# OpenDriveLab/OccNet

Hardware: AMD Instinct MI355X
Metric: nuScenes samples/sec (6-cam 900x1600 -> 200x200x16 voxels) (higher is better)
Workload: dtype f32 hot path (GEMM operands bf16x3-split, SCA value rows q16 block floating point) + bf16 backbone; 1 GPU; bevformer_base_occ forward: 6x(3x928x1600) images -> ResNet-50+FPN -> 4 BEVFormer layers (TSA+SCA+FFN) -> lifter + 2xConv3d decoder -> 200x200x16 voxels x (17 logits + 2 flow); history_frames=0, mode=infer, scope=e2e, input=resident-f32, samples_per_gpu=1, global_batch=1, parallelism=dp1, step_graph=False, linear_precision=bf16x3, backbone_dtype=bf16

## Files before the change

### occnet_amd/csrc/bottleneck64_nhwc_bf16.hip

```cpp
#include "common.h"

namespace occ {

constexpr int kBnTH = 8, kBnTW = 16, kBnHH = 10, kBnHW = 18, kBnNP = kBnHH * kBnHW;
constexpr int kBnXS = 80;
constexpr int kBnXA = 192 * kBnXS;
constexpr int kBnMS = 144;
constexpr int kBnH1ROW = kBnHW * kBnMS;
constexpr int kBnH1 = kBnHH * kBnH1ROW;
constexpr int kBnC2 = 128 * kBnMS;
constexpr int kBnOLD = 256 + 4;

__global__ void mfma_pack_b_frag_kernel(const float* __restrict__ w, unsigned short* __restrict__ packed,
                                        int N, int K) {
  const long n_el = (long)N * K;
  const long idx = (long)blockIdx.x * blockDim.x + threadIdx.x;
  if (idx >= n_el) return;
  const int j = (int)(idx & 7), lane = (int)((idx >> 3) & 63);
  const long rest = idx >> 9;
  const int nts = N / 32;
  const int nt = (int)(rest % nts), ks = (int)(rest / nts);
  const int n = nt * 32 + (lane & 31), k = ks * 16 + (lane >> 5) * 8 + j;
  packed[idx] = bf16_rne(w[(long)n * K + k]);
}

template <int CIN, bool DS>
__global__ __launch_bounds__(256, 2) void bottleneck64_nhwc_bf16_kernel(
    const uint4* __restrict__ x, const uint4* __restrict__ w1p, const float* __restrict__ b1,
    const uint4* __restrict__ w2p, const float* __restrict__ b2, const uint4* __restrict__ w3p,
    const float* __restrict__ b3, unsigned short* __restrict__ out, int H, int W, int tiles_x, int tiles_y) {
  static_assert(CIN % 32 == 0 && (!DS || CIN == 64), "downsample variant keeps both x chunks in LDS");
  constexpr int NCH = CIN / 32, CQ = CIN / 8;
  constexpr int STAGE_BYTES = 2 * kBnXA + kBnH1 + kBnC2;
  __shared__ __attribute__((aligned(16))) char lds[STAGE_BYTES];
  static_assert(32 * kBnOLD * 4 <= 2 * kBnXA + kBnH1, "epilogue transpose aliases the x chunks + c1 halo");
  char* const sH1 = lds + 2 * kBnXA;
  char* const sC2 = sH1 + kBnH1;
  const int tid = threadIdx.x, lane = tid & 63, wave = tid >> 6;
  const int vi = lane & 31, kb = lane >> 5;
  int bid = blockIdx.x;
  const int tx_i = bid % tiles_x; bid /= tiles_x;
  const int ty_i = bid % tiles_y;
  const int img = bid / tiles_y;
  const int y0 = ty_i * kBnTH, x0 = tx_i * kBnTW;

  long hofs0, hofs1, hofs2;
  int hdst0, hdst1, hdst2;
  bool hin0, hin1, hin2, hlive0, hlive1, hlive2;
#define OCC_BN_ROLE(K, OFS, DST, IN, LIVE)                                                        \
  {                                                                                               \
    const int idx = tid + 256 * (K);                                                              \
    LIVE = idx < kBnNP * 4;                                                                       \
    const int p = LIVE ? idx >> 2 : 0, piece = idx & 3;                                           \
    const int hy = p / kBnHW, hx = p % kBnHW;                                                     \
    const int iy = y0 - 1 + hy, ix = x0 - 1 + hx;                                                 \
    IN = LIVE && iy >= 0 && iy < H && ix >= 0 && ix < W;                                          \
    const int cy = min(max(iy, 0), H - 1), cx = min(max(ix, 0), W - 1);                           \
    OFS = (((long)img * H + cy) * W + cx) * CQ + piece;                                           \
    DST = p * kBnXS + piece * 16;                                                                 \
  }
  OCC_BN_ROLE(0, hofs0, hdst0, hin0, hlive0)
  OCC_BN_ROLE(1, hofs1, hdst1, hin1, hlive1)
  OCC_BN_ROLE(2, hofs2, hdst2, hin2, hlive2)
#undef OCC_BN_ROLE
  const unsigned hm0 = hin0 ? 0xffffffffu : 0u, hm1 = hin1 ? 0xffffffffu : 0u, hm2 = hin2 ? 0xffffffffu : 0u;
  uint4 vh0_0, vh1_0, vh2_0, vh0_1, vh1_1, vh2_1, vh0_2, vh1_2, vh2_2, vh0_3, vh1_3, vh2_3;
#define OCC_BN_ISSUE_X(S, CH)                                                                     \
  {                                                                                               \
    const long cq = (long)(CH) * 4;                                                               \
    vh0_##S = x[hofs0 + cq]; vh1_##S = x[hofs1 + cq]; vh2_##S = x[hofs2 + cq];                    \
  }
  const int rot = DS ? 0 : (int)((blockIdx.x * 5u) % (unsigned)NCH);
#define OCC_BN_CH(CI) (((CI) + rot) % NCH)

  const int ntA = wave & 1, mtA0 = 3 * (wave >> 1);
  const int ntB = wave & 1, mtB0 = 2 * (wave >> 1);
  float4 bA[4], bB[4];
#pragma unroll
  for (int g = 0; g < 4; ++g) {
    bA[g] = *reinterpret_cast<const float4*>(b1 + ntA * 32 + 8 * g + 4 * kb);
    bB[g] = *reinterpret_cast<const float4*>(b2 + ntB * 32 + 8 * g + 4 * kb);
  }
  f32x16 acc1[3];
#pragma unroll
  for (int j = 0; j < 3; ++j)
#pragma unroll
    for (int r = 0; r < 16; ++r) acc1[j][r] = 0.f;
  uint4 wa[4][2];
#define OCC_BN_ISSUE_W1(SLOT, CH)                                                                 \
  {                                                                                               \
    wa[SLOT][0] = w1p[(((long)(CH) * 2 + 0) * 2 + ntA) * 64 + lane];                              \
    wa[SLOT][1] = w1p[(((long)(CH) * 2 + 1) * 2 + ntA) * 64 + lane];                              \
  }
#define OCC_BN_ISSUE_XW(S, CH) { OCC_BN_ISSUE_W1(S, CH) OCC_BN_ISSUE_X(S, CH) }
  OCC_BN_ISSUE_XW(0, OCC_BN_CH(0))
  OCC_BN_ISSUE_XW(1, OCC_BN_CH(NCH > 1 ? 1 : 0))
  if (NCH > 2) {
    OCC_BN_ISSUE_XW(2, OCC_BN_CH(NCH > 2 ? 2 : 0))
    OCC_BN_ISSUE_XW(3, OCC_BN_CH(NCH > 3 ? 3 : 0))
  }
#define OCC_BN_STEP_A(S, CI)                                                                      \
  {                                                                                               \
    char* sX = lds + ((CI) & 1) * kBnXA;                                                          \
    if (hlive0) *reinterpret_cast<uint4*>(sX + hdst0) = make_uint4(vh0_##S.x & hm0, vh0_##S.y & hm0, vh0_##S.z & hm0, vh0_##S.w & hm0); \
    if (hlive1) *reinterpret_cast<uint4*>(sX + hdst1) = make_uint4(vh1_##S.x & hm1, vh1_##S.y & hm1, vh1_##S.z & hm1, vh1_##S.w & hm1); \
    if (hlive2) *reinterpret_cast<uint4*>(sX + hdst2) = make_uint4(vh2_##S.x & hm2, vh2_##S.y & hm2, vh2_##S.z & hm2, vh2_##S.w & hm2); \
    const bf16x8 wf0 = __builtin_bit_cast(bf16x8, wa[S][0]), wf1 = __builtin_bit_cast(bf16x8, wa[S][1]); \
    __syncthreads();                                                                              \
    if ((CI) + 4 < NCH) OCC_BN_ISSUE_XW(S, OCC_BN_CH((CI) + 4 < NCH ? (CI) + 4 : NCH - 1))        \
    _Pragma("unroll") for (int j = 0; j < 3; ++j) {                                               \
      const bf16x8 af0 = *reinterpret_cast<const bf16x8*>(sX + ((mtA0 + j) * 32 + vi) * kBnXS + kb * 16);      \
      const bf16x8 af1 = *reinterpret_cast<const bf16x8*>(sX + ((mtA0 + j) * 32 + vi) * kBnXS + 32 + kb * 16); \
      acc1[j] = __builtin_amdgcn_mfma_f32_32x32x16_bf16(wf0, af0, acc1[j], 0, 0, 0);              \
      acc1[j] = __builtin_amdgcn_mfma_f32_32x32x16_bf16(wf1, af1, acc1[j], 0, 0, 0);              \
    }                                                                                             \
  }
#pragma unroll
  for (int ci = 0; ci < NCH; ci += 4) {
    OCC_BN_STEP_A(0, ci)
    if (ci + 1 < NCH) OCC_BN_STEP_A(1, ci + 1)
    if (ci + 2 < NCH) OCC_BN_STEP_A(2, ci + 2)
    if (ci + 3 < NCH) OCC_BN_STEP_A(3, ci + 3)
  }
#undef OCC_BN_STEP_A
#undef OCC_BN_ISSUE_XW
#undef OCC_BN_ISSUE_W1
#undef OCC_BN_ISSUE_X
#undef OCC_BN_CH

  constexpr int PFB = 12;
  uint4 wr[PFB];
#pragma unroll
  for (int s = 0; s < PFB; ++s) wr[s] = w2p[((long)s * 2 + ntB) * 64 + lane];

#pragma unroll
  for (int j = 0; j < 3; ++j) {
    const int p = (mtA0 + j) * 32 + vi;
    const int hy = p / kBnHW, hx = p - hy * kBnHW;
    const int iy = y0 - 1 + hy, ix = x0 - 1 + hx;
    const float m = (iy >= 0 && iy < H && ix >= 0 && ix < W) ? 1.f : 0.f;
    if (p < kBnNP) {
      char* dst = sH1 + p * kBnMS + (ntA * 32 + 4 * kb) * 2;
#pragma unroll
      for (int g = 0; g < 4; ++g) {
        const float v0 = fmaxf(acc1[j][4 * g + 0] + bA[g].x, 0.f) * m, v1 = fmaxf(acc1[j][4 * g + 1] + bA[g].y, 0.f) * m;
        const float v2 = fmaxf(acc1[j][4 * g + 2] + bA[g].z, 0.f) * m, v3 = fmaxf(acc1[j][4 * g + 3] + bA[g].w, 0.f) * m;
        *reinterpret_cast<uint2*>(dst + 16 * g) = make_uint2(pack_bf16x2_rne(v0, v1), pack_bf16x2_rne(v2, v3));
      }
    }
  }
  __syncthreads();

  f32x16 acc2[2];
#pragma unroll
  for (int j = 0; j < 2; ++j)
#pragma unroll
    for (int r = 0; r < 16; ++r) acc2[j][r] = 0.f;
  const int ab0 = (2 * mtB0 + (vi >> 4)) * kBnH1ROW + (vi & 15) * kBnMS + kb * 16;
  const int ab1 = ab0 + 2 * kBnH1ROW;
  {
    bf16x8 a0 = *reinterpret_cast<const bf16x8*>(sH1 + ab0), a1 = *reinterpret_cast<const bf16x8*>(sH1 + ab1);
#pragma unroll
    for (int s = 0; s < 36; ++s) {
      const bf16x8 wf = __builtin_bit_cast(bf16x8, wr[s % PFB]);
      if (s + PFB < 36) wr[s % PFB] = w2p[((long)(s + PFB) * 2 + ntB) * 64 + lane];
      bf16x8 a0n = a0, a1n = a1;
      if (s + 1 < 36) {
        const int tap = (s + 1) >> 2, ks = (s + 1) & 3;
        const int toff = (tap / 3) * kBnH1ROW + (tap % 3) * kBnMS + ks * 32;
        a0n = *reinterpret_cast<const bf16x8*>(sH1 + ab0 + toff);
        a1n = *reinterpret_cast<const bf16x8*>(sH1 + ab1 + toff);
      }
      acc2[0] = __builtin_amdgcn_mfma_f32_32x32x16_bf16(wf, a0, acc2[0], 0, 0, 0);
      acc2[1] = __builtin_amdgcn_mfma_f32_32x32x16_bf16(wf, a1, acc2[1], 0, 0, 0);
      __builtin_amdgcn_sched_barrier(0);
      a0 = a0n; a1 = a1n;
    }
  }
  constexpr int KS3 = DS ? 8 : 4;
  uint4 w3r[4][2];
#define OCC_BN_ISSUE_W3(SLOT, KS)                                                                 \
  {                                                                                               \
    w3r[SLOT][0] = w3p[((long)(KS) * 8 + 2 * wave + 0) * 64 + lane];                              \
    w3r[SLOT][1] = w3p[((long)(KS) * 8 + 2 * wave + 1) * 64 + lane];                              \
  }
  OCC_BN_ISSUE_W3(0, 0)
  OCC_BN_ISSUE_W3(1, 1)
  OCC_BN_ISSUE_W3(2, 2)
  OCC_BN_ISSUE_W3(3, 3)
#pragma unroll
  for (int j = 0; j < 2; ++j) {
    char* dst = sC2 + ((mtB0 + j) * 32 + vi) * kBnMS + (ntB * 32 + 4 * kb) * 2;
#pragma unroll
    for (int g = 0; g < 4; ++g) {
      const float v0 = fmaxf(acc2[j][4 * g + 0] + bB[g].x, 0.f), v1 = fmaxf(acc2[j][4 * g + 1] + bB[g].y, 0.f);
      const float v2 = fmaxf(acc2[j][4 * g + 2] + bB[g].z, 0.f), v3 = fmaxf(acc2[j][4 * g + 3] + bB[g].w, 0.f);
      *reinterpret_cast<uint2*>(dst + 16 * g) = make_uint2(pack_bf16x2_rne(v0, v1), pack_bf16x2_rne(v2, v3));
    }
  }
  __syncthreads();

  f32x16 acc3[4][2];
#pragma unroll
  for (int rt = 0; rt < 4; ++rt)
#pragma unroll
    for (int t = 0; t < 2; ++t)
#pragma unroll
      for (int r = 0; r < 16; ++r) acc3[rt][t][r] = 0.f;
#pragma unroll
  for (int ks = 0; ks < KS3; ++ks) {
    const bf16x8 wf0 = __builtin_bit_cast(bf16x8, w3r[ks & 3][0]);
    const bf16x8 wf1 = __builtin_bit_cast(bf16x8, w3r[ks & 3][1]);
    if (ks + 4 < KS3) OCC_BN_ISSUE_W3(ks & 3, ks + 4)
#pragma unroll
    for (int rt = 0; rt < 4; ++rt) {
      bf16x8 af;
      if (ks < 4) {
        af = *reinterpret_cast<const bf16x8*>(sC2 + (rt * 32 + vi) * kBnMS + ks * 32 + kb * 16);
      } else {
        const int p = (2 * rt + (vi >> 4) + 1) * kBnHW + (vi & 15) + 1;
        af = *reinterpret_cast<const bf16x8*>(lds + ((ks - 4) >> 1) * kBnXA + p * kBnXS + ((ks - 4) & 1) * 32 + kb * 16);
      }
      acc3[rt][0] = __builtin_amdgcn_mfma_f32_32x32x16_bf16(af, wf0, acc3[rt][0], 0, 0, 0);
      acc3[rt][1] = __builtin_amdgcn_mfma_f32_32x32x16_bf16(af, wf1, acc3[rt][1], 0, 0, 0);
    }
  }
#undef OCC_BN_ISSUE_W3

  const int c = lane * 4;
  const float4 bv = *reinterpret_cast<const float4*>(b3 + c);
  float* sO = reinterpret_cast<float*>(lds);
  const unsigned short* xs = reinterpret_cast<const unsigned short*>(x);
  uint2 rv[8], rn[8];
#define OCC_BN_ISSUE_RES(DST, RT)                                                                 \
  _Pragma("unroll") for (int rr = 0; rr < 8; ++rr) {                                              \
    DST[rr] = make_uint2(0u, 0u);                                                                 \
    if (!DS) {                                                                                    \
      const int row = wave * 8 + rr;                                                              \
      const int cy = min(y0 + 2 * (RT) + (row >> 4), H - 1), cx = min(x0 + (row & 15), W - 1);    \
      DST[rr] = *reinterpret_cast<const uint2*>(xs + (((long)img * H + cy) * W + cx) * CIN + c);  \
    }                                                                                             \
  }
  OCC_BN_ISSUE_RES(rn, 0)
#pragma unroll
  for (int rt = 0; rt < 4; ++rt) {
    __syncthreads();
#pragma unroll
    for (int t = 0; t < 2; ++t)
#pragma unroll
      for (int r = 0; r < 16; ++r)
        sO[((r & 3) + 8 * (r >> 2) + 4 * kb) * kBnOLD + (wave * 2 + t) * 32 + vi] = acc3[rt][t][r];
#pragma unroll
    for (int rr = 0; rr < 8; ++rr) rv[rr] = rn[rr];
    if (rt + 1 < 4) OCC_BN_ISSUE_RES(rn, rt + 1)
    __syncthreads();
#pragma unroll
    for (int rr = 0; rr < 8; ++rr) {
      const int row = wave * 8 + rr;
      const int oy = y0 + 2 * rt + (row >> 4), ox = x0 + (row & 15);
      if (oy < H && ox < W) {
        float4 v = *reinterpret_cast<const float4*>(sO + row * kBnOLD + c);
        v.x += bv.x + bf16_to_f32((unsigned short)(rv[rr].x & 0xffffu));
        v.y += bv.y + bf16_to_f32((unsigned short)(rv[rr].x >> 16));
        v.z += bv.z + bf16_to_f32((unsigned short)(rv[rr].y & 0xffffu));
        v.w += bv.w + bf16_to_f32((unsigned short)(rv[rr].y >> 16));
        v.x = fmaxf(v.x, 0.f); v.y = fmaxf(v.y, 0.f); v.z = fmaxf(v.z, 0.f); v.w = fmaxf(v.w, 0.f);
        const uint2 o = make_uint2(pack_bf16x2_rne(v.x, v.y), pack_bf16x2_rne(v.z, v.w));
        *reinterpret_cast<uint2*>(out + (((long)img * H + oy) * W + ox) * 256 + c) = o;
      }
    }
  }
#undef OCC_BN_ISSUE_RES
}

}

extern "C" int occ_mfma_pack_b_frag_bf16(const float* weight, void* packed, int N, int K, void* stream) {
  using namespace occ;
  OCC_CHECK_ARG(weight && packed, "mfma_pack_b_frag_bf16: null pointer argument");
  OCC_CHECK_ARG(N > 0 && K > 0, "mfma_pack_b_frag_bf16: bad dimension");
  if (N % 32 || K % 16) {
    set_error("mfma_pack_b_frag_bf16: N=%d K=%d (need N %% 32 == 0, K %% 16 == 0)", N, K);
    return OCC_E_UNSUPPORTED;
  }
  const long n = (long)N * K;
  hipLaunchKernelGGL(mfma_pack_b_frag_kernel, dim3((unsigned)((n + 255) / 256)), dim3(256), 0,
                     reinterpret_cast<hipStream_t>(stream), weight, reinterpret_cast<unsigned short*>(packed),
                     N, K);
  OCC_CHECK_LAUNCH("mfma_pack_b_frag_bf16");
  return OCC_OK;
}

extern "C" int occ_bottleneck64_nhwc_bf16(const void* x, const void* w1_frag, const float* b1,
                                          const void* w2_frag, const float* b2, const void* w3_frag,
                                          const float* b3, void* out, int batch, int H, int W, int Cin,
                                          int downsample, void* stream) {
  using namespace occ;
  OCC_CHECK_ARG(x && w1_frag && b1 && w2_frag && b2 && w3_frag && b3 && out,
                "bottleneck64_nhwc_bf16: null pointer argument");
  OCC_CHECK_ARG(batch > 0 && H > 0 && W > 0, "bottleneck64_nhwc_bf16: bad dimension");
  if (!((Cin == 256 && !downsample) || (Cin == 64 && downsample))) {
    set_error("bottleneck64_nhwc_bf16: no kernel for Cin=%d downsample=%d (256/identity or 64/projection)", Cin,
              downsample);
    return OCC_E_UNSUPPORTED;
  }
  const int tiles_x = (W + kBnTW - 1) / kBnTW, tiles_y = (H + kBnTH - 1) / kBnTH;
  hipStream_t st = reinterpret_cast<hipStream_t>(stream);
  const unsigned gx = (unsigned)((long)batch * tiles_x * tiles_y);
#define OCC_BN_LAUNCH(CINN, DSS)                                                                     \
  hipLaunchKernelGGL((bottleneck64_nhwc_bf16_kernel<CINN, DSS>), dim3(gx), dim3(256), 0, st,            \
                     reinterpret_cast<const uint4*>(x), reinterpret_cast<const uint4*>(w1_frag), b1,    \
                     reinterpret_cast<const uint4*>(w2_frag), b2, reinterpret_cast<const uint4*>(w3_frag), \
                     b3, reinterpret_cast<unsigned short*>(out), H, W, tiles_x, tiles_y)
  if (downsample) OCC_BN_LAUNCH(64, true); else OCC_BN_LAUNCH(256, false);
#undef OCC_BN_LAUNCH
  OCC_CHECK_LAUNCH("bottleneck64_nhwc_bf16");
  return OCC_OK;
}
```

### occnet_amd/csrc/common.h

```cpp
#pragma once
#include <hip/hip_runtime.h>
#include <stdint.h>
#include <stdio.h>
#include <stdlib.h>
#include "../../include/occnet_amd.h"

namespace occ {

void set_error(const char* fmt, ...);
#define OCC_CHECK_ARG(cond, ...)              \
  do {                                        \
    if (!(cond)) {                            \
      ::occ::set_error(__VA_ARGS__);          \
      return OCC_E_INVALID;                   \
    }                                         \
  } while (0)
#define OCC_CHECK_LAUNCH(what)                                                  \
  do {                                                                          \
    hipError_t e__ = hipGetLastError();                                         \
    if (e__ != hipSuccess) {                                                    \
      ::occ::set_error("%s: launch failed: %s", what, hipGetErrorString(e__));  \
      return OCC_E_LAUNCH;                                                      \
    }                                                                           \
  } while (0)
// ... 107 lines not shown
  __builtin_amdgcn_wave_barrier();
  __builtin_amdgcn_fence(__ATOMIC_ACQUIRE, "wavefront");
}

template <int UNROLL>
__device__ __forceinline__ float4 gather_samples(const float* __restrict__ vb,
                                                 const SampleParam* sp, int ns, float4 acc) {
  int s = 0;
  for (; s + UNROLL <= ns; s += UNROLL) {
    float4 w[UNROLL];
    int4 o[UNROLL];
#pragma unroll
    for (int u = 0; u < UNROLL; ++u) {
      w[u] = *reinterpret_cast<const float4*>(sp[s + u].w);
      o[u] = *reinterpret_cast<const int4*>(sp[s + u].o);
    }
    float4 v[UNROLL][4];
#pragma unroll
    for (int u = 0; u < UNROLL; ++u) {
      v[u][0] = *reinterpret_cast<const float4*>(vb + o[u].x);
      v[u][1] = *reinterpret_cast<const float4*>(vb + o[u].y);
      v[u][2] = *reinterpret_cast<const float4*>(vb + o[u].z);
      v[u][3] = *reinterpret_cast<const float4*>(vb + o[u].w);
    }
#pragma unroll
    for (int u = 0; u < UNROLL; ++u) {
      const float ww[4] = {w[u].x, w[u].y, w[u].z, w[u].w};
#pragma unroll
      for (int k = 0; k < 4; ++k) {
        acc.x = fmaf(ww[k], v[u][k].x, acc.x);
        acc.y = fmaf(ww[k], v[u][k].y, acc.y);
        acc.z = fmaf(ww[k], v[u][k].z, acc.z);
        acc.w = fmaf(ww[k], v[u][k].w, acc.w);
      }
    }
  }
  for (; s < ns; ++s) {
    const float4 w = *reinterpret_cast<const float4*>(sp[s].w);
    const int4 o = *reinterpret_cast<const int4*>(sp[s].o);
    const float4 v0 = *reinterpret_cast<const float4*>(vb + o.x);
    const float4 v1 = *reinterpret_cast<const float4*>(vb + o.y);
    const float4 v2 = *reinterpret_cast<const float4*>(vb + o.z);
    const float4 v3 = *reinterpret_cast<const float4*>(vb + o.w);
    acc.x = fmaf(w.x, v0.x, acc.x); acc.y = fmaf(w.x, v0.y, acc.y);
    acc.z = fmaf(w.x, v0.z, acc.z); acc.w = fmaf(w.x, v0.w, acc.w);
    acc.x = fmaf(w.y, v1.x, acc.x); acc.y = fmaf(w.y, v1.y, acc.y);
    acc.z = fmaf(w.y, v1.z, acc.z); acc.w = fmaf(w.y, v1.w, acc.w);
    acc.x = fmaf(w.z, v2.x, acc.x); acc.y = fmaf(w.z, v2.y, acc.y);
    acc.z = fmaf(w.z, v2.z, acc.z); acc.w = fmaf(w.z, v2.w, acc.w);
    acc.x = fmaf(w.w, v3.x, acc.x); acc.y = fmaf(w.w, v3.y, acc.y);
    acc.z = fmaf(w.w, v3.z, acc.z); acc.w = fmaf(w.w, v3.w, acc.w);
  }
  return acc;
}

constexpr unsigned kOobOffset = 0x7fffff00u;

struct __attribute__((aligned(16))) SampleParamB {
  float w[4];
  unsigned o[4];
};

__device__ __forceinline__ int bilinear_setup_b(float loc_x, float loc_y, float attn, int H, int W, int lvl_pix0,
                                                unsigned pix_bytes, unsigned dead, int live, SampleParamB& sp) {
  const BilinearTerms t = bilinear_terms(loc_x, loc_y, H, W, live);
  const int base = lvl_pix0 + t.h_low * W + t.w_low;
  sp.w[0] = t.c[0] ? t.hh * t.hw * attn : 0.f; sp.o[0] = t.c[0] ? (unsigned)base * pix_bytes : dead;
  sp.w[1] = t.c[1] ? t.hh * t.lw * attn : 0.f; sp.o[1] = t.c[1] ? (unsigned)(base + 1) * pix_bytes : dead;
  sp.w[2] = t.c[2] ? t.lh * t.hw * attn : 0.f; sp.o[2] = t.c[2] ? (unsigned)(base + W) * pix_bytes : dead;
  sp.w[3] = t.c[3] ? t.lh * t.lw * attn : 0.f; sp.o[3] = t.c[3] ? (unsigned)(base + W + 1) * pix_bytes : dead;
  return t.c[0] + t.c[1] + t.c[2] + t.c[3];
}

__device__ __forceinline__ __amdgpu_buffer_rsrc_t uniform_rsrc(const void* base, unsigned bytes) {
  const unsigned long long a = reinterpret_cast<unsigned long long>(base);
  const unsigned lo = __builtin_amdgcn_readfirstlane((unsigned)a);
  const unsigned hi = __builtin_amdgcn_readfirstlane((unsigned)(a >> 32));
  void* p = reinterpret_cast<void*>(((unsigned long long)hi << 32) | lo);
  return __builtin_amdgcn_make_buffer_rsrc(p, 0, (int)__builtin_amdgcn_readfirstlane(bytes), 0x00020000);
}

__device__ __forceinline__ void block_lds_sync() { asm volatile("s_waitcnt lgkmcnt(0)\n\ts_barrier" ::: "memory"); }

__device__ __forceinline__ float4 buf_load16(__amdgpu_buffer_rsrc_t rsrc, unsigned byte_off) {
  return __builtin_bit_cast(float4, __builtin_amdgcn_raw_buffer_load_b128(rsrc, (int)byte_off, 0, 0));
}

__device__ __forceinline__ void fma4(float4& acc, float w, const float4& v) {
  acc.x = fmaf(w, v.x, acc.x); acc.y = fmaf(w, v.y, acc.y);
  acc.z = fmaf(w, v.z, acc.z); acc.w = fmaf(w, v.w, acc.w);
}

template <int UNROLL>
__device__ __forceinline__ float4 gather_samples_buf(__amdgpu_buffer_rsrc_t rsrc, unsigned lane_off,
                                                     const SampleParamB* sp, int ns, float4 acc) {
  int s = 0;
  for (; s + UNROLL <= ns; s += UNROLL) {
    float4 v[UNROLL][4];
#pragma unroll
    for (int u = 0; u < UNROLL; ++u) {
      const occ_u32x4 o = *reinterpret_cast<const occ_u32x4*>(sp[s + u].o);
#pragma unroll
      for (int k = 0; k < 4; ++k) v[u][k] = buf_load16(rsrc, o[k] + lane_off);
    }
#pragma unroll
    for (int u = 0; u < UNROLL; ++u) {
      const float4 w = *reinterpret_cast<const float4*>(sp[s + u].w);
      fma4(acc, w.x, v[u][0]); fma4(acc, w.y, v[u][1]); fma4(acc, w.z, v[u][2]); fma4(acc, w.w, v[u][3]);
    }
  }
  for (; s < ns; ++s) {
    const occ_u32x4 o = *reinterpret_cast<const occ_u32x4*>(sp[s].o);
    const float4 w = *reinterpret_cast<const float4*>(sp[s].w);
    float4 v[4];
#pragma unroll
    for (int k = 0; k < 4; ++k) v[k] = buf_load16(rsrc, o[k] + lane_off);
    fma4(acc, w.x, v[0]); fma4(acc, w.y, v[1]); fma4(acc, w.z, v[2]); fma4(acc, w.w, v[3]);
  }
  return acc;
}

__device__ __forceinline__ void fma_mix_lo(float& acc, float w, unsigned packed) {
  asm("v_fma_mix_f32 %0, %1, %2, %0 op_sel_hi:[0,1,0]" : "+v"(acc) : "v"(w), "v"(packed));
}
__device__ __forceinline__ void fma_mix_hi(float& acc, float w, unsigned packed) {
  asm("v_fma_mix_f32 %0, %1, %2, %0 op_sel:[0,1,0] op_sel_hi:[0,1,0]" : "+v"(acc) : "v"(w), "v"(packed));
}

__device__ __forceinline__ void fma8h(float4& acc, float4& acc2, float w, const float4& raw) {
  const occ_u32x4 h = __builtin_bit_cast(occ_u32x4, raw);
  fma_mix_lo(acc.x, w, h[0]); fma_mix_hi(acc.y, w, h[0]); fma_mix_lo(acc.z, w, h[1]); fma_mix_hi(acc.w, w, h[1]);
  fma_mix_lo(acc2.x, w, h[2]); fma_mix_hi(acc2.y, w, h[2]); fma_mix_lo(acc2.z, w, h[3]); fma_mix_hi(acc2.w, w, h[3]);
}

__device__ __forceinline__ void fma8q(float4& acc, float4& acc2, float w, const float4& raw) {
  typedef float occ_f32x2 __attribute__((ext_vector_type(2)));
  const occ_u32x4 h = __builtin_bit_cast(occ_u32x4, raw);
  const unsigned e = (h[0] & 3u) | ((h[0] >> 14) & 12u);
  const float ws = ldexpf(w, (int)e);
  const occ_f32x2 ww = {ws, ws};
  occ_f32x2 a0 = {acc.x, acc.y}, a1 = {acc.z, acc.w}, a2 = {acc2.x, acc2.y}, a3 = {acc2.z, acc2.w};
  const occ_f32x2 v0 = {(float)(short)(h[0] & 0xffffu), (float)((int)h[0] >> 16)};
  const occ_f32x2 v1 = {(float)(short)(h[1] & 0xffffu), (float)((int)h[1] >> 16)};
  const occ_f32x2 v2 = {(float)(short)(h[2] & 0xffffu), (float)((int)h[2] >> 16)};
  const occ_f32x2 v3 = {(float)(short)(h[3] & 0xffffu), (float)((int)h[3] >> 16)};
  a0 = __builtin_elementwise_fma(v0, ww, a0);
  a1 = __builtin_elementwise_fma(v1, ww, a1);
  a2 = __builtin_elementwise_fma(v2, ww, a2);
  a3 = __builtin_elementwise_fma(v3, ww, a3);
  acc = make_float4(a0[0], a0[1], a1[0], a1[1]);
  acc2 = make_float4(a2[0], a2[1], a3[0], a3[1]);
}

constexpr float kQ16Magic = 12582912.f;
__device__ __forceinline__ int q16_group_exponent(float m, int eosc) {
  const int x = __builtin_amdgcn_frexp_expf(m * 1.000244140625f) + eosc;
  const int E = x < 0 ? 0 : x > 15 ? 15 : x;
  return m > 0.f ? E : 0;
}
__device__ __forceinline__ unsigned q16_rne_bits(float y) { return __float_as_uint(y + kQ16Magic); }
__device__ __forceinline__ unsigned q16_pack_lo16(unsigned lo, unsigned hi) { return __builtin_amdgcn_perm(hi, lo, 0x05040100u); }
__device__ __forceinline__ unsigned q16_pair(float v0, float v1, float f) {
  return q16_pack_lo16(q16_rne_bits(v0 * f), q16_rne_bits(v1 * f));
}
__device__ __forceinline__ unsigned q16_pair_tagged(float v0, float v1, float fS, float c0, float c1, int r0, int r1, int sh) {
  const unsigned q0 = (q16_rne_bits(fmaf(v0, fS, c0)) << sh) + (unsigned)r0;
// ... 43 lines not shown
```

### occnet_amd/csrc/conv3d_mfma.hip

```cpp
#include "heads_x3.h"

namespace occ {

template <int Z, int CH, int TY, int TX>
struct ConvGeom {
  static_assert(32 % Z == 0 && Z % 4 == 0, "Z must be 4, 8, 16 or 32");
  static_assert(CH == 8 || CH == 16, "CH must be 8 or 16");
  static constexpr int PX = 32 / Z;
  static_assert(TX % PX == 0, "TX must be a multiple of the pillars per row tile");
  static constexpr int VS = CH + 4;
  static constexpr int PS = ((Z + 2) * VS + 63) / 64 * 64;
  static constexpr int HX = TX + 2, HY = TY + 2;
  static constexpr int LDS_FLOATS = HY * HX * PS;
  static constexpr int ROW_TILES = TY * TX / PX;
  static_assert(ROW_TILES % 4 == 0, "row tiles must split over 4 waves");
  static constexpr int NACC = ROW_TILES / 4;
  static constexpr int TXG = TX / PX;
};

struct ConvTile { int b, y0, x0; };
template <int TY, int TX>
__device__ __forceinline__ ConvTile conv_tile_of_block(int tiles_x, int tiles_y) {
  int bid;
  {
    const int n = (int)gridDim.x, q = n >> 3, r = n & 7, x = (int)blockIdx.x & 7, j = (int)blockIdx.x >> 3;
    bid = x * q + (x < r ? x : r) + j;
  }
  const int tx_i = bid % tiles_x;
  bid /= tiles_x;
  const int ty_i = bid % tiles_y;
  return {bid / tiles_y, ty_i * TY, tx_i * TX};
}

template <int Z, int CH, int TY, int TX, int LAYOUT>
__global__ __launch_bounds__(256) void conv3d_mfma_kernel(
    const float* __restrict__ in, const float* __restrict__ wp, const float* __restrict__ scale,
    const float* __restrict__ shift, float* __restrict__ out, int Y, int X, int Cin, long out_sb,
    long out_sy, long out_sx, int relu, int tiles_x, int tiles_y) {
  using G = ConvGeom<Z, CH, TY, TX>;
  constexpr int VS = G::VS, PS = G::PS, HX = G::HX, HY = G::HY, NACC = G::NACC, H2 = CH / 2;
  extern __shared__ __attribute__((aligned(16))) float lds[];
  const int tid = threadIdx.x, lane = tid & 63, wave = tid >> 6;
  const ConvTile tile = conv_tile_of_block<TY, TX>(tiles_x, tiles_y);
  const int b = tile.b, y0 = tile.y0, x0 = tile.x0;
  const float* inb = in + (long)b * Y * X * Z * Cin;

  for (int i = tid; i < HY * HX * 2 * VS; i += 256) {
    const int pil = i / (2 * VS), rem = i % (2 * VS);
    lds[pil * PS + (rem >= VS ? (Z + 1) * VS : 0) + rem % VS] = 0.f;
  }

  f32x16 acc[NACC];
#pragma unroll
  for (int a = 0; a < NACC; ++a)
#pragma unroll
    for (int r = 0; r < 16; ++r) acc[a][r] = 0.f;

  const int vi = lane & 31, kh = lane >> 5;
  int abase[NACC];
#pragma unroll
  for (int a = 0; a < NACC; ++a) {
    const int rt = wave * NACC + a;
    const int ty = rt / G::TXG, txg = rt % G::TXG;
    const int px = txg * G::PX + vi / Z, z = vi % Z;
    abase[a] = (ty * HX + px) * PS + z * VS + kh * H2;
  }

  const int nph = Cin / CH;
  for (int p = 0; p < nph; ++p) {
    if (p) __syncthreads();
    if (LAYOUT == 0) {
      constexpr int PARTS = CH / 4, ITEMS = HY * HX * Z * PARTS, ITERS = (ITEMS + 255) / 256;
      float4 v[ITERS];
#pragma unroll
      for (int it = 0; it < ITERS; ++it) {
        const int idx = tid + it * 256;
        const int part = idx % PARTS, z = (idx / PARTS) % Z, pil = idx / (PARTS * Z);
        const int gy = y0 + pil / HX - 1, gx = x0 + pil % HX - 1;
        v[it] = make_float4(0.f, 0.f, 0.f, 0.f);
        if (idx < ITEMS && gy >= 0 && gy < Y && gx >= 0 && gx < X)
          v[it] = *reinterpret_cast<const float4*>(inb + (((long)gy * X + gx) * Z + z) * Cin +
                                                   p * CH + part * 4);
      }
#pragma unroll
      for (int it = 0; it < ITERS; ++it) {
        const int idx = tid + it * 256;
        const int part = idx % PARTS, z = (idx / PARTS) % Z, pil = idx / (PARTS * Z);
        if (idx < ITEMS)
          *reinterpret_cast<float4*>(lds + pil * PS + (z + 1) * VS + part * 4) = v[it];
      }
    } else {
      constexpr int Z4 = Z / 4, ITEMS = HY * HX * CH * Z4, ITERS = (ITEMS + 255) / 256;
      float4 v[ITERS];
#pragma unroll
      for (int it = 0; it < ITERS; ++it) {
        const int idx = tid + it * 256;
        const int z4 = idx % Z4, ci = (idx / Z4) % CH, pil = idx / (Z4 * CH);
        const int gy = y0 + pil / HX - 1, gx = x0 + pil % HX - 1;
        v[it] = make_float4(0.f, 0.f, 0.f, 0.f);
        if (idx < ITEMS && gy >= 0 && gy < Y && gx >= 0 && gx < X)
          v[it] = *reinterpret_cast<const float4*>(inb + ((long)gy * X + gx) * Z * Cin +
                                                   (long)(p * CH + ci) * Z + z4 * 4);
      }
#pragma unroll
      for (int it = 0; it < ITERS; ++it) {
        const int idx = tid + it * 256;
        const int z4 = idx % Z4, ci = (idx / Z4) % CH, pil = idx / (Z4 * CH);
        if (idx < ITEMS) {
          float* d = lds + pil * PS + (z4 * 4 + 1) * VS + ci;
          d[0] = v[it].x; d[VS] = v[it].y; d[2 * VS] = v[it].z; d[3 * VS] = v[it].w;
// ... 870 lines not shown
```

Baseline: 184.0 samples/s.

## Stream bottleneck input via direct-to-LDS DMA and reuse identity from LDS

Replaces register-staged halo loads in the fused ResNet bottleneck kernel with global_load_lds DMA into a 4-deep swizzled LDS ring. The residual identity is taken from the already-staged input chunks instead of being re-read from global memory, and biases are staged in LDS. The epilogue now writes through a per-wave scratch with wave-local syncs instead of block barriers. Tiles are also remapped for XCD locality. The aim is to cut register pressure, redundant global reads and block-level syncs, at the cost of more complex inline-asm DMA and a swizzle that must stay consistent everywhere.

```diff
diff --git a/occnet_amd/csrc/bottleneck64_nhwc_bf16.hip b/occnet_amd/csrc/bottleneck64_nhwc_bf16.hip
--- a/occnet_amd/csrc/bottleneck64_nhwc_bf16.hip
+++ b/occnet_amd/csrc/bottleneck64_nhwc_bf16.hip
@@ -3,13 +3,16 @@
 namespace occ {
 
 constexpr int kBnTH = 8, kBnTW = 16, kBnHH = 10, kBnHW = 18, kBnNP = kBnHH * kBnHW;
-constexpr int kBnXS = 80;
+constexpr int kBnXS = 64;
 constexpr int kBnXA = 192 * kBnXS;
+constexpr int kBnNXB = 4;
 constexpr int kBnMS = 144;
 constexpr int kBnH1ROW = kBnHW * kBnMS;
 constexpr int kBnH1 = kBnHH * kBnH1ROW;
 constexpr int kBnC2 = 128 * kBnMS;
-constexpr int kBnOLD = 256 + 4;
+constexpr int kBnEP = 144, kBnES = 32 * kBnEP;
+constexpr int kBnLds = kBnNXB * kBnXA + kBnH1 + (64 + 64 + 256) * 4;
+static_assert(2 * kBnXA + kBnC2 <= kBnNXB * kBnXA && 4 * kBnES <= kBnH1, "c2 / the scratch alias dead buffers");
 
 __global__ void mfma_pack_b_frag_kernel(const float* __restrict__ w, unsigned short* __restrict__ packed,
                                         int N, int K) {
@@ -24,108 +27,125 @@
   packed[idx] = bf16_rne(w[(long)n * K + k]);
 }
 
+__device__ __forceinline__ float bn_relu(float v) { return v < 0.f ? 0.f : v; }
+
+__device__ __forceinline__ void bn_dma16(const uint4* src, unsigned lds_dst) {
+  unsigned keep;
+  asm volatile("s_mov_b32 %0, m0\n\ts_mov_b32 m0, %2\n\ts_nop 0\n\tglobal_load_lds_dwordx4 %1, off\n\ts_mov_b32 m0, %0"
+               : "=&s"(keep)
+               : "v"(src), "s"(lds_dst)
+               : "memory");
+}
+template <int N>
+__device__ __forceinline__ void bn_wait_dma() { asm volatile("s_waitcnt vmcnt(%0)" ::"n"(N) : "memory"); }
+
 template <int CIN, bool DS>
 __global__ __launch_bounds__(256, 2) void bottleneck64_nhwc_bf16_kernel(
     const uint4* __restrict__ x, const uint4* __restrict__ w1p, const float* __restrict__ b1,
     const uint4* __restrict__ w2p, const float* __restrict__ b2, const uint4* __restrict__ w3p,
     const float* __restrict__ b3, unsigned short* __restrict__ out, int H, int W, int tiles_x, int tiles_y) {
-  static_assert(CIN % 32 == 0 && (!DS || CIN == 64), "downsample variant keeps both x chunks in LDS");
+  static_assert(CIN % 64 == 0 && CIN <= 256 && (!DS || CIN == 64), "downsample variant keeps both x chunks in LDS");
   constexpr int NCH = CIN / 32, CQ = CIN / 8;
-  constexpr int STAGE_BYTES = 2 * kBnXA + kBnH1 + kBnC2;
-  __shared__ __attribute__((aligned(16))) char lds[STAGE_BYTES];
-  static_assert(32 * kBnOLD * 4 <= 2 * kBnXA + kBnH1, "epilogue transpose aliases the x chunks + c1 halo");
-  char* const sH1 = lds + 2 * kBnXA;
-  char* const sC2 = sH1 + kBnH1;
+  __shared__ __attribute__((aligned(16))) char lds[kBnLds];
+  char* const sH1 = lds + kBnNXB * kBnXA;
+  char* const sC2 = lds + 2 * kBnXA;
+  float* const sBias = reinterpret_cast<float*>(sH1 + kBnH1);
   const int tid = threadIdx.x, lane = tid & 63, wave = tid >> 6;
   const int vi = lane & 31, kb = lane >> 5;
-  int bid = blockIdx.x;
+  const int tile = xcd_local_tile_id();
+  int bid = tile;
   const int tx_i = bid % tiles_x; bid /= tiles_x;
   const int ty_i = bid % tiles_y;
   const int img = bid / tiles_y;
   const int y0 = ty_i * kBnTH, x0 = tx_i * kBnTW;
 
-  long hofs0, hofs1, hofs2;
-  int hdst0, hdst1, hdst2;
-  bool hin0, hin1, hin2, hlive0, hlive1, hlive2;
-#define OCC_BN_ROLE(K, OFS, DST, IN, LIVE)                                                        \
+  long hofs[3];
+#pragma unroll
+  for (int k = 0; k < 3; ++k) {
+    const int item = (4 * k + wave) * 64 + lane;
+    const int p = min(item >> 2, kBnNP - 1), s = item & 3;
+    const int hy = p / kBnHW, hx = p % kBnHW;
+    const int cy = min(max(y0 - 1 + hy, 0), H - 1), cx = min(max(x0 - 1 + hx, 0), W - 1);
+    hofs[k] = (((long)img * H + cy) * W + cx) * CQ + (s ^ (((item >> 2) >> 3) & 3));
+  }
+  const int wave_u = __builtin_amdgcn_readfirstlane(wave);
+  const unsigned xbuf0 = (unsigned)(unsigned long)(__attribute__((address_space(3))) char*)lds + (unsigned)wave_u * 1024u;
+  const int rot = DS ? 0 : (int)(((unsigned)tile * 5u) % (unsigned)NCH);
+#define OCC_BN_CH(CI) (((CI) + rot) % NCH)
+#define OCC_BN_DMA(CI)                                                                            \
   {                                                                                               \
-    const int idx = tid + 256 * (K);                                                              \
-    LIVE = idx < kBnNP * 4;                                                                       \
-    const int p = LIVE ? idx >> 2 : 0, piece = idx & 3;                                           \
-    const int hy = p / kBnHW, hx = p % kBnHW;                                                     \
-    const int iy = y0 - 1 + hy, ix = x0 - 1 + hx;                                                 \
-    IN = LIVE && iy >= 0 && iy < H && ix >= 0 && ix < W;                                          \
-    const int cy = min(max(iy, 0), H - 1), cx = min(max(ix, 0), W - 1);                           \
-    OFS = (((long)img * H + cy) * W + cx) * CQ + piece;                                           \
-    DST = p * kBnXS + piece * 16;                                                                 \
-  }
-  OCC_BN_ROLE(0, hofs0, hdst0, hin0, hlive0)
-  OCC_BN_ROLE(1, hofs1, hdst1, hin1, hlive1)
-  OCC_BN_ROLE(2, hofs2, hdst2, hin2, hlive2)
-#undef OCC_BN_ROLE
-  const unsigned hm0 = hin0 ? 0xffffffffu : 0u, hm1 = hin1 ? 0xffffffffu : 0u, hm2 = hin2 ? 0xffffffffu : 0u;
-  uint4 vh0_0, vh1_0, vh2_0, vh0_1, vh1_1, vh2_1, vh0_2, vh1_2, vh2_2, vh0_3, vh1_3, vh2_3;
-#define OCC_BN_ISSUE_X(S, CH)                                                                     \
-  {                                                                                               \
-    const long cq = (long)(CH) * 4;                                                               \
-    vh0_##S = x[hofs0 + cq]; vh1_##S = x[hofs1 + cq]; vh2_##S = x[hofs2 + cq];                    \
-  }
-  const int rot = DS ? 0 : (int)((blockIdx.x * 5u) % (unsigned)NCH);
-#define OCC_BN_CH(CI) (((CI) + rot) % NCH)
+    const long cq = (long)OCC_BN_CH(CI) * 4;                                                      \
+    const unsigned d = xbuf0 + (unsigned)(((CI) & (kBnNXB - 1)) * kBnXA);                         \
+    bn_dma16(x + hofs[0] + cq, d);                                                                \
+    bn_dma16(x + hofs[1] + cq, d + 4096u);                                                        \
+    bn_dma16(x + hofs[2] + cq, d + 8192u);                                                        \
+  }
 
   const int ntA = wave & 1, mtA0 = 3 * (wave >> 1);
   const int ntB = wave & 1, mtB0 = 2 * (wave >> 1);
-  float4 bA[4], bB[4];
-#pragma unroll
-  for (int g = 0; g < 4; ++g) {
-    bA[g] = *reinterpret_cast<const float4*>(b1 + ntA * 32 + 8 * g + 4 * kb);
-    bB[g] = *reinterpret_cast<const float4*>(b2 + ntB * 32 + 8 * g + 4 * kb);
-  }
+  float4 bias_in = make_float4(0.f, 0.f, 0.f, 0.f);
+  if (tid < 96) bias_in = *reinterpret_cast<const float4*>(tid < 16 ? b1 + 4 * tid : tid < 32 ? b2 + 4 * (tid - 16) : b3 + 4 * (tid - 32));
+  uint4 wa[NCH][2];
+#pragma unroll
+  for (int ci = 0; ci < NCH; ++ci) {
+    wa[ci][0] = w1p[(((long)OCC_BN_CH(ci) * 2 + 0) * 2 + ntA) * 64 + lane];
+    wa[ci][1] = w1p[(((long)OCC_BN_CH(ci) * 2 + 1) * 2 + ntA) * 64 + lane];
+  }
+  OCC_BN_DMA(0)
+  OCC_BN_DMA(1)
+  if (NCH > 2) OCC_BN_DMA(2)
+
   f32x16 acc1[3];
 #pragma unroll
   for (int j = 0; j < 3; ++j)
 #pragma unroll
     for (int r = 0; r < 16; ++r) acc1[j][r] = 0.f;
-  uint4 wa[4][2];
-#define OCC_BN_ISSUE_W1(SLOT, CH)                                                                 \
+  uint2 idt[2][16];
+  if (!DS) {
+#pragma unroll
+    for (int i = 0; i < 32; ++i) idt[i >> 4][i & 15] = make_uint2(0u, 0u);
+  }
+  const int pc0 = ((vi >> 4) + 1) * kBnHW + (vi & 15) + 1;
+  const int fragA = mtA0 * 32 * kBnXS + vi * kBnXS, swzA = (vi >> 3) & 3;
+#define OCC_BN_STEP_A(CI)                                                                         \
   {                                                                                               \
-    wa[SLOT][0] = w1p[(((long)(CH) * 2 + 0) * 2 + ntA) * 64 + lane];                              \
-    wa[SLOT][1] = w1p[(((long)(CH) * 2 + 1) * 2 + ntA) * 64 + lane];                              \
-  }
-#define OCC_BN_ISSUE_XW(S, CH) { OCC_BN_ISSUE_W1(S, CH) OCC_BN_ISSUE_X(S, CH) }
-  OCC_BN_ISSUE_XW(0, OCC_BN_CH(0))
-  OCC_BN_ISSUE_XW(1, OCC_BN_CH(NCH > 1 ? 1 : 0))
-  if (NCH > 2) {
-    OCC_BN_ISSUE_XW(2, OCC_BN_CH(NCH > 2 ? 2 : 0))
-    OCC_BN_ISSUE_XW(3, OCC_BN_CH(NCH > 3 ? 3 : 0))
-  }
-#define OCC_BN_STEP_A(S, CI)                                                                      \
-  {                                                                                               \
-    char* sX = lds + ((CI) & 1) * kBnXA;                                                          \
-    if (hlive0) *reinterpret_cast<uint4*>(sX + hdst0) = make_uint4(vh0_##S.x & hm0, vh0_##S.y & hm0, vh0_##S.z & hm0, vh0_##S.w & hm0); \
-    if (hlive1) *reinterpret_cast<uint4*>(sX + hdst1) = make_uint4(vh1_##S.x & hm1, vh1_##S.y & hm1, vh1_##S.z & hm1, vh1_##S.w & hm1); \
-    if (hlive2) *reinterpret_cast<uint4*>(sX + hdst2) = make_uint4(vh2_##S.x & hm2, vh2_##S.y & hm2, vh2_##S.z & hm2, vh2_##S.w & hm2); \
-    const bf16x8 wf0 = __builtin_bit_cast(bf16x8, wa[S][0]), wf1 = __builtin_bit_cast(bf16x8, wa[S][1]); \
-    __syncthreads();                                                                              \
-    if ((CI) + 4 < NCH) OCC_BN_ISSUE_XW(S, OCC_BN_CH((CI) + 4 < NCH ? (CI) + 4 : NCH - 1))        \
+     \
+         \
+    bn_wait_dma<3 * ((NCH - 1 - (CI)) < 2 ? (NCH - 1 - (CI)) : 2)>();                             \
+    block_lds_sync();                                                                             \
+    if ((CI) + 3 < NCH) OCC_BN_DMA((CI) + 3 < NCH ? (CI) + 3 : 0)                                 \
+    const char* sX = lds + ((CI) & (kBnNXB - 1)) * kBnXA;                                         \
+    const bf16x8 wf0 = __builtin_bit_cast(bf16x8, wa[CI][0]), wf1 = __builtin_bit_cast(bf16x8, wa[CI][1]); \
     _Pragma("unroll") for (int j = 0; j < 3; ++j) {                                               \
-      const bf16x8 af0 = *reinterpret_cast<const bf16x8*>(sX + ((mtA0 + j) * 32 + vi) * kBnXS + kb * 16);      \
-      const bf16x8 af1 = *reinterpret_cast<const bf16x8*>(sX + ((mtA0 + j) * 32 + vi) * kBnXS + 32 + kb * 16); \
+      const bf16x8 af0 = *reinterpret_cast<const bf16x8*>(sX + fragA + j * (32 * kBnXS) + ((kb ^ swzA) << 4));       \
+      const bf16x8 af1 = *reinterpret_cast<const bf16x8*>(sX + fragA + j * (32 * kBnXS) + (((2 + kb) ^ swzA) << 4)); \
       acc1[j] = __builtin_amdgcn_mfma_f32_32x32x16_bf16(wf0, af0, acc1[j], 0, 0, 0);              \
       acc1[j] = __builtin_amdgcn_mfma_f32_32x32x16_bf16(wf1, af1, acc1[j], 0, 0, 0);              \
     }                                                                                             \
-  }
-#pragma unroll
-  for (int ci = 0; ci < NCH; ci += 4) {
-    OCC_BN_STEP_A(0, ci)
-    if (ci + 1 < NCH) OCC_BN_STEP_A(1, ci + 1)
-    if (ci + 2 < NCH) OCC_BN_STEP_A(2, ci + 2)
-    if (ci + 3 < NCH) OCC_BN_STEP_A(3, ci + 3)
+    if (!DS && (OCC_BN_CH(CI) >> 1) == wave_u) {                                                  \
+      _Pragma("unroll") for (int rt = 0; rt < 4; ++rt) {                                          \
+        const int pc = pc0 + 2 * kBnHW * rt;                                                      \
+        _Pragma("unroll") for (int q = 0; q < 4; ++q)                                             \
+          idt[(CI) & 1][4 * rt + q] =                                                             \
+              *reinterpret_cast<const uint2*>(sX + pc * kBnXS + ((q ^ ((pc >> 3) & 3)) << 4) + 8 * kb); \
+      }                                                                                           \
+    }                                                                                             \
+    if ((CI) == 0 && tid < 96) *reinterpret_cast<float4*>(sBias + 4 * tid) = bias_in;             \
+  }
+  OCC_BN_STEP_A(0)
+  OCC_BN_STEP_A(1)
+  if (NCH > 2) {
+    OCC_BN_STEP_A(NCH > 2 ? 2 : 0)
+    OCC_BN_STEP_A(NCH > 2 ? 3 : 0)
+  }
+  if (NCH > 4) {
+    OCC_BN_STEP_A(NCH > 4 ? 4 : 0)
+    OCC_BN_STEP_A(NCH > 4 ? 5 : 0)
+    OCC_BN_STEP_A(NCH > 4 ? 6 : 0)
+    OCC_BN_STEP_A(NCH > 4 ? 7 : 0)
   }
 #undef OCC_BN_STEP_A
-#undef OCC_BN_ISSUE_XW
-#undef OCC_BN_ISSUE_W1
-#undef OCC_BN_ISSUE_X
+#undef OCC_BN_DMA
 #undef OCC_BN_CH
 
   constexpr int PFB = 12;
@@ -138,18 +158,19 @@
     const int p = (mtA0 + j) * 32 + vi;
     const int hy = p / kBnHW, hx = p - hy * kBnHW;
     const int iy = y0 - 1 + hy, ix = x0 - 1 + hx;
-    const float m = (iy >= 0 && iy < H && ix >= 0 && ix < W) ? 1.f : 0.f;
+    const int in = lane_flag(iy >= 0) & lane_flag(iy < H) & lane_flag(ix >= 0) & lane_flag(ix < W);
     if (p < kBnNP) {
       char* dst = sH1 + p * kBnMS + (ntA * 32 + 4 * kb) * 2;
 #pragma unroll
       for (int g = 0; g < 4; ++g) {
-        const float v0 = fmaxf(acc1[j][4 * g + 0] + bA[g].x, 0.f) * m, v1 = fmaxf(acc1[j][4 * g + 1] + bA[g].y, 0.f) * m;
-        const float v2 = fmaxf(acc1[j][4 * g + 2] + bA[g].z, 0.f) * m, v3 = fmaxf(acc1[j][4 * g + 3] + bA[g].w, 0.f) * m;
+        const float4 bA = *reinterpret_cast<const float4*>(sBias + ntA * 32 + 8 * g + 4 * kb);
+        const float v0 = in ? bn_relu(acc1[j][4 * g + 0] + bA.x) : 0.f, v1 = in ? bn_relu(acc1[j][4 * g + 1] + bA.y) : 0.f;
+        const float v2 = in ? bn_relu(acc1[j][4 * g + 2] + bA.z) : 0.f, v3 = in ? bn_relu(acc1[j][4 * g + 3] + bA.w) : 0.f;
         *reinterpret_cast<uint2*>(dst + 16 * g) = make_uint2(pack_bf16x2_rne(v0, v1), pack_bf16x2_rne(v2, v3));
       }
     }
   }
-  __syncthreads();
+  block_lds_sync();
 
   f32x16 acc2[2];
 #pragma unroll
@@ -193,12 +214,13 @@
     char* dst = sC2 + ((mtB0 + j) * 32 + vi) * kBnMS + (ntB * 32 + 4 * kb) * 2;
 #pragma unroll
     for (int g = 0; g < 4; ++g) {
-      const float v0 = fmaxf(acc2[j][4 * g + 0] + bB[g].x, 0.f), v1 = fmaxf(acc2[j][4 * g + 1] + bB[g].y, 0.f);
-      const float v2 = fmaxf(acc2[j][4 * g + 2] + bB[g].z, 0.f), v3 = fmaxf(acc2[j][4 * g + 3] + bB[g].w, 0.f);
+      const float4 bB = *reinterpret_cast<const float4*>(sBias + 64 + ntB * 32 + 8 * g + 4 * kb);
+      const float v0 = bn_relu(acc2[j][4 * g + 0] + bB.x), v1 = bn_relu(acc2[j][4 * g + 1] + bB.y);
+      const float v2 = bn_relu(acc2[j][4 * g + 2] + bB.z), v3 = bn_relu(acc2[j][4 * g + 3] + bB.w);
       *reinterpret_cast<uint2*>(dst + 16 * g) = make_uint2(pack_bf16x2_rne(v0, v1), pack_bf16x2_rne(v2, v3));
     }
   }
-  __syncthreads();
+  block_lds_sync();
 
   f32x16 acc3[4][2];
 #pragma unroll
@@ -218,59 +240,50 @@
       if (ks < 4) {
         af = *reinterpret_cast<const bf16x8*>(sC2 + (rt * 32 + vi) * kBnMS + ks * 32 + kb * 16);
       } else {
-        const int p = (2 * rt + (vi >> 4) + 1) * kBnHW + (vi & 15) + 1;
-        af = *reinterpret_cast<const bf16x8*>(lds + ((ks - 4) >> 1) * kBnXA + p * kBnXS + ((ks - 4) & 1) * 32 + kb * 16);
+        const int pc = pc0 + 2 * kBnHW * rt;
+        af = *reinterpret_cast<const bf16x8*>(lds + ((ks - 4) >> 1) * kBnXA + pc * kBnXS +
+                                              (((((ks - 4) & 1) * 2 + kb) ^ ((pc >> 3) & 3)) << 4));
       }
-      acc3[rt][0] = __builtin_amdgcn_mfma_f32_32x32x16_bf16(af, wf0, acc3[rt][0], 0, 0, 0);
-      acc3[rt][1] = __builtin_amdgcn_mfma_f32_32x32x16_bf16(af, wf1, acc3[rt][1], 0, 0, 0);
+      acc3[rt][0] = __builtin_amdgcn_mfma_f32_32x32x16_bf16(wf0, af, acc3[rt][0], 0, 0, 0);
+      acc3[rt][1] = __builtin_amdgcn_mfma_f32_32x32x16_bf16(wf1, af, acc3[rt][1], 0, 0, 0);
     }
   }
 #undef OCC_BN_ISSUE_W3
 
-  const int c = lane * 4;
-  const float4 bv = *reinterpret_cast<const float4*>(b3 + c);
-  float* sO = reinterpret_cast<float*>(lds);
-  const unsigned short* xs = reinterpret_cast<const unsigned short*>(x);
-  uint2 rv[8], rn[8];
-#define OCC_BN_ISSUE_RES(DST, RT)                                                                 \
-  _Pragma("unroll") for (int rr = 0; rr < 8; ++rr) {                                              \
-    DST[rr] = make_uint2(0u, 0u);                                                                 \
-    if (!DS) {                                                                                    \
-      const int row = wave * 8 + rr;                                                              \
-      const int cy = min(y0 + 2 * (RT) + (row >> 4), H - 1), cx = min(x0 + (row & 15), W - 1);    \
-      DST[rr] = *reinterpret_cast<const uint2*>(xs + (((long)img * H + cy) * W + cx) * CIN + c);  \
-    }                                                                                             \
-  }
-  OCC_BN_ISSUE_RES(rn, 0)
+  char* const scratch = sH1 + wave * kBnES;
+  const float* const sB3 = sBias + 128 + wave * 64 + 4 * kb;
+  const bool odd = rot & 1;
+  const int erow = lane >> 3, epiece = lane & 7;
 #pragma unroll
   for (int rt = 0; rt < 4; ++rt) {
-    __syncthreads();
 #pragma unroll
     for (int t = 0; t < 2; ++t)
 #pragma unroll
-      for (int r = 0; r < 16; ++r)
-        sO[((r & 3) + 8 * (r >> 2) + 4 * kb) * kBnOLD + (wave * 2 + t) * 32 + vi] = acc3[rt][t][r];
-#pragma unroll
-    for (int rr = 0; rr < 8; ++rr) rv[rr] = rn[rr];
-    if (rt + 1 < 4) OCC_BN_ISSUE_RES(rn, rt + 1)
-    __syncthreads();
-#pragma unroll
-    for (int rr = 0; rr < 8; ++rr) {
-      const int row = wave * 8 + rr;
+      for (int q = 0; q < 4; ++q) {
+        const float4 bv = *reinterpret_cast<const float4*>(sB3 + t * 32 + 8 * q);
+        uint2 id = make_uint2(0u, 0u);
+        if (!DS) {
+          const uint2 ia = idt[t][4 * rt + q], ib = idt[t ^ 1][4 * rt + q];
+          id = make_uint2(odd ? ib.x : ia.x, odd ? ib.y : ia.y);
+        }
+        const float v0 = bn_relu(acc3[rt][t][4 * q + 0] + (bv.x + bf16_lo_to_f32(id.x)));
+        const float v1 = bn_relu(acc3[rt][t][4 * q + 1] + (bv.y + bf16_hi_to_f32(id.x)));
+        const float v2 = bn_relu(acc3[rt][t][4 * q + 2] + (bv.z + bf16_lo_to_f32(id.y)));
+        const float v3 = bn_relu(acc3[rt][t][4 * q + 3] + (bv.w + bf16_hi_to_f32(id.y)));
+        *reinterpret_cast<uint2*>(scratch + vi * kBnEP + t * 64 + 16 * q + 8 * kb) =
+            make_uint2(pack_bf16x2_rne(v0, v1), pack_bf16x2_rne(v2, v3));
+      }
+    wave_lds_sync();
+#pragma unroll
+    for (int j = 0; j < 4; ++j) {
+      const int row = erow + 8 * j;
       const int oy = y0 + 2 * rt + (row >> 4), ox = x0 + (row & 15);
-      if (oy < H && ox < W) {
-        float4 v = *reinterpret_cast<const float4*>(sO + row * kBnOLD + c);
-        v.x += bv.x + bf16_to_f32((unsigned short)(rv[rr].x & 0xffffu));
-        v.y += bv.y + bf16_to_f32((unsigned short)(rv[rr].x >> 16));
-        v.z += bv.z + bf16_to_f32((unsigned short)(rv[rr].y & 0xffffu));
-        v.w += bv.w + bf16_to_f32((unsigned short)(rv[rr].y >> 16));
-        v.x = fmaxf(v.x, 0.f); v.y = fmaxf(v.y, 0.f); v.z = fmaxf(v.z, 0.f); v.w = fmaxf(v.w, 0.f);
-        const uint2 o = make_uint2(pack_bf16x2_rne(v.x, v.y), pack_bf16x2_rne(v.z, v.w));
-        *reinterpret_cast<uint2*>(out + (((long)img * H + oy) * W + ox) * 256 + c) = o;
-      }
-    }
-  }
-#undef OCC_BN_ISSUE_RES
+      const uint4 v = *reinterpret_cast<const uint4*>(scratch + row * kBnEP + epiece * 16);
+      if (oy < H && ox < W)
+        *reinterpret_cast<uint4*>(out + (((long)img * H + oy) * W + ox) * 256 + wave * 64 + epiece * 8) = v;
+    }
+    wave_lds_sync();
+  }
 }
 
 }
diff --git a/occnet_amd/csrc/common.h b/occnet_amd/csrc/common.h
--- a/occnet_amd/csrc/common.h
+++ b/occnet_amd/csrc/common.h
@@ -213,6 +213,11 @@
 
 __device__ __forceinline__ void block_lds_sync() { asm volatile("s_waitcnt lgkmcnt(0)\n\ts_barrier" ::: "memory"); }
 
+__device__ __forceinline__ int xcd_local_tile_id() {
+  const int n = (int)gridDim.x, q = n >> 3, r = n & 7, x = (int)blockIdx.x & 7, j = (int)blockIdx.x >> 3;
+  return x * q + (x < r ? x : r) + j;
+}
+
 __device__ __forceinline__ float4 buf_load16(__amdgpu_buffer_rsrc_t rsrc, unsigned byte_off) {
   return __builtin_bit_cast(float4, __builtin_amdgcn_raw_buffer_load_b128(rsrc, (int)byte_off, 0, 0));
 }
diff --git a/occnet_amd/csrc/conv3d_mfma.hip b/occnet_amd/csrc/conv3d_mfma.hip
--- a/occnet_amd/csrc/conv3d_mfma.hip
+++ b/occnet_amd/csrc/conv3d_mfma.hip
@@ -21,11 +21,7 @@
 struct ConvTile { int b, y0, x0; };
 template <int TY, int TX>
 __device__ __forceinline__ ConvTile conv_tile_of_block(int tiles_x, int tiles_y) {
-  int bid;
-  {
-    const int n = (int)gridDim.x, q = n >> 3, r = n & 7, x = (int)blockIdx.x & 7, j = (int)blockIdx.x >> 3;
-    bid = x * q + (x < r ? x : r) + j;
-  }
+  int bid = xcd_local_tile_id();
   const int tx_i = bid % tiles_x;
   bid /= tiles_x;
   const int ty_i = bid % tiles_y;
```

After: 184.6 samples/s (median of 6 runs). Within noise of the previous version (+0.3%).
